# Lakonik/MVEdit

Measured on AMD Instinct MI355X. Metric: multi-view denoise-steps/sec (32 views, 512^2), higher is better.
Workload: dtype f16; 1 GPU; 32-view 512x512 get_noise_pred: 64 SD-1.5 UNet forwards (64x64 latents, ctx 77x768) + CFG per step; ControlNet residuals zero; views=32, latent=64, cfg=True, parallelism=views/1

## Files before the change

include/mvedit_amd.h:

```cpp
#ifndef MVEDIT_AMD_H
#define MVEDIT_AMD_H

#include <stdint.h>
#include <stddef.h>

#ifdef __cplusplus
extern "C" {
#endif

#define MVE_API __attribute__((visibility("default")))

typedef enum {
    MVE_OK = 0,
    MVE_ERR_ARG = -1,
    MVE_ERR_HIP = -2,
    MVE_ERR_STATE = -3,
    MVE_ERR_NOMEM = -4
} mve_status;

typedef enum {
    MVE_F32 = 0,
    MVE_F16 = 1,
    MVE_BF16 = 2,
    MVE_I32 = 3,
// ... 8 lines not shown
MVE_API int mve_near_far_from_aabb(const float* d_rays_o, const float* d_rays_d, const float* d_aabb,
                                   uint32_t N, float min_near, float* d_nears, float* d_fars, void* stream);

MVE_API int mve_morton3d(const int32_t* d_coords, uint32_t N, int32_t* d_indices, void* stream);
MVE_API int mve_morton3d_invert(const int32_t* d_indices, uint32_t N, int32_t* d_coords, void* stream);

MVE_API int mve_packbits(const float* d_grid, uint32_t n_bytes, float density_thresh, uint8_t* d_bitfield, void* stream);

MVE_API int mve_flatten_rays(const int32_t* d_rays, uint32_t N, uint32_t M, int32_t* d_res, void* stream);

MVE_API size_t mve_march_scratch_bytes(uint32_t N);
MVE_API int mve_march_rays_train_count(const float* d_rays_o, const float* d_rays_d, const uint8_t* d_grid,
                                       float bound, int contract, float dt_gamma, uint32_t max_steps,
                                       uint32_t N, uint32_t C, uint32_t H,
                                       const float* d_nears, const float* d_fars, const float* d_noises,
                                       int32_t* d_rays, int32_t* d_total, void* d_scratch, void* stream);
MVE_API int mve_march_rays_train_write(const float* d_rays_o, const float* d_rays_d, const uint8_t* d_grid,
                                       float bound, int contract, float dt_gamma, uint32_t max_steps,
                                       uint32_t N, uint32_t C, uint32_t H,
                                       const float* d_nears, const float* d_fars, const float* d_noises,
                                       const int32_t* d_rays, uint32_t capacity,
                                       float* d_xyzs, float* d_dirs, float* d_ts, void* stream);

MVE_API int mve_march_rays_train_clamp(const int32_t* d_rays, uint32_t N, const int32_t* d_total, uint32_t capacity,
                                       int32_t* d_n_samples, int32_t* d_count, int32_t* d_overflow, void* stream);

MVE_API int mve_composite_rays_train_forward(const float* d_sigmas, const float* d_rgbs, const float* d_ts,
                                             const int32_t* d_rays, uint32_t M, uint32_t N, float T_thresh, int binarize,
                                             float* d_weights, float* d_weights_sum, float* d_depth, float* d_image,
                                             void* stream);
MVE_API int mve_composite_rays_train_backward(const float* d_grad_weights, const float* d_grad_weights_sum,
                                              const float* d_grad_depth, const float* d_grad_image,
                                              const float* d_sigmas, const float* d_rgbs, const float* d_ts,
                                              const int32_t* d_rays, const float* d_weights_sum, const float* d_depth,
                                              const float* d_image, uint32_t M, uint32_t N, float T_thresh, int binarize,
                                              float* d_grad_sigmas, float* d_grad_rgbs, void* stream);

MVE_API int mve_march_rays(uint32_t n_alive, uint32_t n_step, const int32_t* d_rays_alive, const float* d_rays_t,
                           const float* d_rays_o, const float* d_rays_d, float bound, int contract, float dt_gamma,
                           uint32_t max_steps, uint32_t C, uint32_t H, const uint8_t* d_grid,
                           const float* d_nears, const float* d_fars,
                           float* d_xyzs, float* d_dirs, float* d_ts, const float* d_noises, void* stream);
MVE_API int mve_composite_rays(uint32_t n_alive, uint32_t n_step, float T_thresh, int binarize,
                               int32_t* d_rays_alive, float* d_rays_t, const float* d_sigmas, const float* d_rgbs,
                               const float* d_ts, float* d_weights_sum, float* d_depth, float* d_image, void* stream);

MVE_API int mve_compact_alive(const int32_t* d_rays_alive, uint32_t n_alive, int32_t* d_out, int32_t* d_n_out,
                              void* d_scratch, void* stream);

MVE_API size_t mve_cull_scratch_bytes(uint32_t M);
MVE_API int mve_cull_samples(const float* d_weights, uint32_t M, float threshold, const int32_t* d_rays, uint32_t N,
                             const float* d_xyzs, const float* d_dirs, const float* d_ts, float* d_out_xyzs, float* d_out_dirs,
                             float* d_out_ts, int32_t* d_out_rays, int32_t* d_pref, int32_t* d_n_out, void* d_scratch,
                             void* stream);
MVE_API int mve_cull_samples_n(const float* d_weights, uint32_t capacity, const int32_t* d_count, float threshold, const int32_t* d_rays,
                               uint32_t N, const float* d_xyzs, const float* d_dirs, const float* d_ts, float* d_out_xyzs,
                               float* d_out_dirs, float* d_out_ts, int32_t* d_out_rays, int32_t* d_pref, int32_t* d_n_out,
                               void* d_scratch, void* stream);

MVE_API int mve_density_grid_points(const int32_t* d_coords, const float* d_noise, uint32_t N, uint32_t grid_size, float bound,
                                    float* d_xyzs, int32_t* d_indices, void* stream);
MVE_API size_t mve_density_grid_scratch_bytes(uint32_t n_cells);
MVE_API int mve_density_grid_update(float* d_density_grid, float* d_tmp_grid, uint32_t n_cells, const float* d_sigmas,
                                    const int32_t* d_indices, uint32_t N, float decay, float* d_mean_density, void* d_scratch,
                                    void* stream);


#define MVE_GEMM_GEGLU   1
#define MVE_GEMM_OUT_F32 2
#define MVE_CONV_W_CHUNK64 4
#define MVE_GEMM_NO_SPLITK 8
#define MVE_CONV_PAD_BR 32
#define MVE_GEMM_RES_AFTER_SCALE 16

MVE_API int mve_gemm(int dtype, const void* d_A, int lda, const void* d_W, int ldw, void* d_out, int ldc,
                     int M, int N, int K, const float* d_bias, const float* d_rowvec, int ldrv, int rows_per_vec,
                     const void* d_residual, int ldr, int flags, float out_scale, void* d_workspace,
                     size_t workspace_bytes, int rows_per_image, void* stream);

MVE_API int mve_gemm_tune(int big_min_blocks);
MVE_API int mve_gemm_red_tune(int on);
MVE_API int mve_gemm_deep_tune(int max_blocks);
MVE_API int mve_gemm_effective_splitk(int M, int N, int K, int rows_per_image);
#define MVE_PLAN_RESIDUAL 1
#define MVE_PLAN_RESIDUAL_LO 2
#define MVE_PLAN_OUT_LO 4
#define MVE_PLAN_ROWVEC 8
#define MVE_PLAN_LN 16
#define MVE_PLAN_BIAS 32
#define MVE_PLAN_WORKSPACE 64
#define MVE_PLAN_SCALED 128
#define MVE_PLAN_DESCRIBE_INTS 12
MVE_API int mve_gemm_plan_describe(int kind, int M, int N, int K, int rows_per_image, int flags, int features, const int* conv_geom, int* out);

MVE_API int mve_gemm_pp_profile(void* d_buf);

MVE_API size_t mve_gemm_workspace_bytes(int M, int N, int K, int rows_per_image);

MVE_API int mve_conv3x3(int dtype, const void* d_x1, int C1, const void* d_x2, int C2, int B, int Hs, int Ws,
                        int stride, int upsample, const void* d_W, int Cout, void* d_out, int ldc,
                        const float* d_bias, const float* d_rowvec, int ldrv, const void* d_residual, int ldr,
                        int flags, float out_scale, void* d_workspace, size_t workspace_bytes, void* stream);

MVE_API int mve_conv3x3_shortcut(int dtype, const void* x1, int C1, const void* x3, int C3, const void* x4, int C4, int B, int Hs,
                                 int Ws, const void* W, int Cout, void* out, int ldc, const float* bias, const float* bias2,
                                 const void* residual, int ldr, int flags, float out_scale, void* d_workspace,
                                 size_t workspace_bytes, void* stream);

MVE_API int mve_upsample_conv_phases_supported(int C, int Cout, int B, int Hs, int Ws);
MVE_API int mve_upsample_conv_phases_tune(int one_launch);
MVE_API size_t mve_upsample_conv_phases_workspace_bytes(int C, int Cout, int B, int Hs, int Ws);
MVE_API int mve_pack_upsample_phase_weights(int src_dtype, int dst_dtype, const void* d_w_oihw, int Cout, int C, void* d_W4, void* stream);
MVE_API int mve_upsample_conv_phases(int dtype, const void* d_x, int C, int B, int Hs, int Ws, const void* d_W4, int Cout, void* d_out,
                                     const float* d_bias, int flags, void* d_workspace, size_t workspace_bytes, void* d_out_lo, void* stream);

MVE_API int mve_gemm_pair(int dtype, const void* d_A, int lda, const void* d_W, int ldw, void* d_out, int ldc,
                          int M, int N, int K, const float* d_bias, const float* d_rowvec, int ldrv, int rows_per_vec,
                          const void* d_residual, int ldr, int flags, float out_scale, void* d_workspace,
                          size_t workspace_bytes, int rows_per_image, const void* d_residual_lo, void* d_out_lo, void* stream);

MVE_API int mve_gemm_pair_ln(int dtype, const void* d_A, int lda, const void* d_W, int ldw, void* d_out, int ldc, int M, int N, int K,
                             const float* d_bias, const void* d_residual, int ldr, void* d_workspace, size_t workspace_bytes, int rows_per_image,
                             const void* d_residual_lo, void* d_out_lo, void* d_ln_out, int ld_ln, const float* d_ln_gamma, const float* d_ln_beta,
                             float ln_eps, void* stream);
MVE_API int mve_gemm_ln_fuse_tune(int on);

MVE_API int mve_conv3x3_pair(int dtype, const void* x1, int C1, const void* x2, int C2, int B, int Hs, int Ws, int stride,
                             int upsample, const void* W, int Cout, void* out, int ldc, const float* bias, const float* rowvec,
                             int ldrv, const void* residual, int ldr, int flags, float out_scale, void* d_workspace,
                             size_t workspace_bytes, const void* d_residual_lo, void* d_out_lo, void* stream);
MVE_API int mve_conv3x3_shortcut_pair(int dtype, const void* x1, int C1, const void* x3, int C3, const void* x4, int C4, int B, int Hs,
                                      int Ws, const void* W, int Cout, void* out, int ldc, const float* bias, const float* bias2,
                                      int flags, float out_scale, void* d_workspace, size_t workspace_bytes, void* d_out_lo, void* stream);
MVE_API int mve_groupnorm_silu_pair(int dtype, const void* d_x1, int C1, const void* d_x2, int C2, int B, int HW, int G,
                                    float eps, const float* d_gamma, const float* d_beta, int silu, void* d_out,
                                    void* d_workspace, const void* d_x1_lo, const void* d_x2_lo, void* stream);
MVE_API int mve_layernorm_pair(int dtype, const void* d_x, int ldx, void* d_y, int ldy, int M, int C,
                               const float* d_gamma, const float* d_beta, float eps, const void* d_x_lo, void* stream);
MVE_API int mve_axpy_pair(int dtype, const void* d_a, const void* d_a_lo, const void* d_b, float alpha, void* d_y, void* d_y_lo, size_t n, void* stream);

MVE_API int mve_mxfp8_packed_k(int K);
MVE_API int mve_mxfp8_quantize(int dtype, const void* d_x, int ldx, int R, int K, uint8_t* d_q, uint8_t* d_e, void* stream);
MVE_API int mve_mxfp8_gemm(const uint8_t* d_aq, const uint8_t* d_ae, const uint8_t* d_wq, const uint8_t* d_we, int M, int N, int K, int out_dtype,
                           void* d_out, int ldc, const float* d_bias, const void* d_residual, int ldr, void* stream);

MVE_API int mve_attention(int dtype, const void* d_Q, int ldq, const void* d_K, int ldk, const void* d_V, int ldv,
                          const void* d_K2, int ldk2, const void* d_V2, int ldv2, void* d_O, int ldo,
                          int B, int Lq, int Lk, int Lk2, int heads, int head_dim, float scale, void* stream);
MVE_API int mve_attention_tune(int variant);
MVE_API int mve_attention_profile(unsigned long long* out4);
MVE_API int mve_attention_prescaled(int dtype, const void* d_Q, int ldq, const void* d_K, int ldk, const void* d_V, int ldv,
                                    const void* d_K2, int ldk2, const void* d_V2, int ldv2, void* d_O, int ldo,
                                    int B, int Lq, int Lk, int Lk2, int heads, int head_dim, void* stream);


MVE_API int mve_attention_causal(int dtype, const void* d_Q, int ldq, const void* d_K, int ldk, const void* d_V, int ldv, void* d_O, int ldo,
                                 int B, int L, int heads, int head_dim, float scale, void* stream);
MVE_API int mve_clip_embed(int dtype, const int32_t* d_ids, const void* d_tok, const void* d_pos, void* d_out, int B, int L, int C, int vocab,
                           int max_pos, void* stream);
#define MVE_ACT_QUICK_GELU 0
#define MVE_ACT_GELU 1
MVE_API int mve_act(int dtype, int kind, const void* d_x, void* d_y, size_t n, void* stream);
MVE_API int mve_clip_pool(int dtype, const void* d_x, const int32_t* d_ids, void* d_out, int B, int L, int C, int eos_token_id, void* stream);


MVE_API int mve_clip_patchify(int dtype, const void* d_pixels, int B, int H, int W, int P, void* d_rows, int ld, void* stream);
MVE_API int mve_clip_vision_embed(int dtype, const void* d_patch, const void* d_cls, const void* d_pos, void* d_out, int B, int G2, int C, void* stream);


MVE_API int mve_dpt_stem_rows(int dtype, const void* d_pixels, int B, int S, void* d_rows, int ld, void* stream);
MVE_API int mve_dpt_maxpool(int dtype, const void* d_x, int B, int H, int W, int C, void* d_y, void* stream);
MVE_API int mve_dpt_gather_s2(int dtype, const void* d_x, int B, int H, int W, int C, void* d_y, void* stream);
MVE_API int mve_dpt_upsample2x(int dtype, const void* d_x, int B, int H, int W, int C, void* d_y, void* stream);
MVE_API int mve_dpt_add_relu(int dtype, const void* d_a, const void* d_b, void* d_y, size_t n, void* stream);


MVE_API int mve_loftr_stem_rows(int dtype, const void* d_pixels, int B, int H, int W, void* d_rows, int ld, void* stream);
MVE_API int mve_loftr_leaky_relu(int dtype, const void* d_x, void* d_y, size_t n, float slope, void* stream);
MVE_API int mve_loftr_pos_add(int dtype, const void* d_x, const float* d_pos, void* d_y, int B, int HW, int C, void* stream);

MVE_API size_t mve_linattn_workspace_bytes(int B, int S, int H, int D);
MVE_API int mve_linattn_kv(int dtype, const void* d_k, int ldk, const void* d_v, int ldv, int B, int S, int H, int D, float* d_kv, void* d_workspace,
                           size_t workspace_bytes, void* stream);
MVE_API int mve_linattn_apply(int dtype, const void* d_q, int ldq, const float* d_kv, void* d_out, int ldo, int B, int L, int H, int D, float eps,
                              void* stream);

MVE_API int mve_dsmax_stats(const float* d_sim, int N, int L, int S, int ld, float* d_row_stats, float* d_col_stats, void* stream);
MVE_API int mve_dsmax_conf(const float* d_sim, int N, int L, int S, int ld, const float* d_row_stats, const float* d_col_stats, float* d_conf, void* stream);
MVE_API size_t mve_dsmax_select_workspace_bytes(int N, int L, int S);
MVE_API int mve_dsmax_select(const float* d_conf, int N, int H0, int W0, int H1, int W1, float thr, int border, float scale, int64_t* d_b_ids,
                             int64_t* d_i_ids, int64_t* d_j_ids, float* d_mconf, float* d_mkpts0_c, float* d_mkpts1_c, int* d_count, void* d_workspace,
                             size_t workspace_bytes, void* stream);

MVE_API int mve_loftr_unfold(int dtype, const void* d_feat, int N, int Hf, int Wf, int C, const int64_t* d_b_ids, const int64_t* d_ids, int M, void* d_rows,
                             void* stream);
MVE_API int mve_loftr_ln_add(int dtype, const void* d_o, int ldo, const void* d_x, int ldx, void* d_y, int ldy, int M, int C, const float* d_gamma,
                             const float* d_beta, float eps, void* stream);
MVE_API int mve_loftr_gather_rows(int dtype, const void* d_feat, int N, int L, int C, const int64_t* d_b_ids, const int64_t* d_ids, int M, void* d_rows,
                                  void* stream);
MVE_API int mve_loftr_fine_match(int dtype, const void* d_feat0, const void* d_feat1, int M, int C, const float* d_mkpts1_c, float radius, float* d_expec_f,
                                 float* d_mkpts1_f, void* stream);


MVE_API int mve_attention_relpos(int dtype, const void* d_Q, int ldq, const void* d_K, int ldk, const void* d_V, int ldv, const void* d_rel_h,
                                 const void* d_rel_w, void* d_O, int ldo, int NS, int gh, int gw, int heads, int head_dim, float scale, void* stream);
MVE_API int mve_sam_window_partition(int dtype, const void* d_x, int B, int G, int C, int window, void* d_win, void* stream);
MVE_API int mve_sam_window_unpartition(int dtype, const void* d_win, int B, int G, int C, int window, void* d_x, void* stream);
MVE_API int mve_sam_pos_add(int dtype, const void* d_x, const void* d_pos, void* d_y, int B, int HW, int C, void* stream);

MVE_API int mve_groupnorm_tune(int fused_max_hw);
MVE_API size_t mve_groupnorm_workspace_bytes(int B, int HW, int C, int G);
MVE_API int mve_groupnorm_silu(int dtype, const void* d_x1, int C1, const void* d_x2, int C2, int B, int HW, int G,
                               float eps, const float* d_gamma, const float* d_beta, int silu, void* d_out,
                               void* d_workspace, void* stream);

MVE_API int mve_layernorm(int dtype, const void* d_x, int ldx, void* d_y, int ldy, int M, int C,
                          const float* d_gamma, const float* d_beta, float eps, void* stream);

MVE_API int mve_nchw_to_nhwc(int dst_dtype, int src_dtype, const void* d_x, int B, int C, int H, int W, int Cpad,
                             void* d_y, void* stream);
MVE_API int mve_nhwc_to_nchw(int dst_dtype, int src_dtype, const void* d_x, int ld, int B, int C, int H, int W,
                             void* d_y, void* stream);
MVE_API int mve_timestep_embedding(int dtype, const float* d_t, int B, int dim, void* d_out, void* stream);
MVE_API int mve_text_time_embedding(int dtype, const void* d_text_embeds, int text_dtype, int text_dim, const float* d_time_ids, int n_ids,
                                    int time_embed_dim, int B, void* d_out, void* stream);
MVE_API int mve_silu(int dtype, const void* d_x, void* d_y, size_t n, void* stream);
MVE_API int mve_axpy(int dtype, const void* d_a, const void* d_b, float alpha, void* d_y, size_t n, void* stream);
MVE_API int mve_softmax_rows(int dtype, const float* d_scores, size_t lds, int M, int N, void* d_probs, size_t ldp, void* stream);
MVE_API int mve_cfg_combine(const float* d_uncond, const float* d_text, float guidance_scale, float* d_out, size_t n,
                            void* stream);
MVE_API int mve_x0_prediction(const float* d_latents_scaled, const float* d_noise_pred, float sqrt_alpha_bar,
                              float sqrt_one_minus_alpha_bar, size_t n, float* d_x0, void* stream);

MVE_API int mve_tonemap_lut(const float* d_x, size_t n, const float* d_lut_x, const float* d_lut_y, int steps, int inverse, int linear,
                            float* d_out, void* stream);
MVE_API int mve_tonemap_lut_backward(const float* d_x, const float* d_grad_out, size_t n, const float* d_lut_x, const float* d_lut_y,
                                     int steps, int inverse, int linear, float* d_grad_x, void* stream);

MVE_API int mve_gaussian_blur(const float* d_x, int planes, int H, int W, int ksize, float sigma, int adjoint, const float* d_base,
                              float offset, float* d_tmp, float* d_out, void* stream);

MVE_API int mve_sh_encode(const float* d_inputs, uint32_t B, int degree, float* d_outputs, float* d_dy_dx, void* stream);
MVE_API int mve_sh_encode_backward(const float* d_grad, const float* d_dy_dx, uint32_t B, int degree, float* d_grad_inputs, void* stream);
MVE_API int mve_shade_views(const float* d_rgba, const float* d_normal_fg, const float* d_cam_lights, uint32_t n_views,
                            uint32_t pix_per_view, float ambient_light, float bg_color, const float* d_lut_x, const float* d_lut_y,
                            int steps, float* d_image, void* stream);
MVE_API int mve_shade_points(const float* d_albedo, const float* d_normal, const float* d_lights, size_t N, float ambient_light,
                             const float* d_lut_x, const float* d_lut_y, int steps, float* d_out, const float* d_grad_out,
                             float* d_grad_albedo, float* d_grad_normal, void* stream);

typedef struct MveReconLossDesc {
    int32_t P, ps, shaded, is_init, lut_steps;
    float ambient_light, bg_color, normal_bg[3];
    float pixel_loss_weight, normal_reg_weight, depth_weight, entropy_weight, bg_width;
    const float *d_lut_x, *d_lut_y;
    const float *d_image, *d_weights_sum, *d_depth;
    const float *d_weights, *d_ts;
    uint32_t M;
    const float *d_target_dir, *d_target_rgbs, *d_target_m, *d_target_n, *d_target_depth;
    const float *d_patch_w, *d_patch_lights;
} MveReconLossDesc;
MVE_API size_t mve_recon_loss_workspace_bytes(int P, int ps, uint32_t M);
MVE_API int mve_recon_loss_forward(const MveReconLossDesc* desc, void* d_ws, size_t ws_bytes, float* d_losses, float* d_out_rgbs,
                                   float* d_out_normals, void* stream);
MVE_API int mve_recon_loss_backward(const MveReconLossDesc* desc, void* d_ws, size_t ws_bytes, const float* d_g_out_rgbs,
                                    const float* d_g_out_normals, const float* d_g_loss, float* d_g_image, float* d_g_weights_sum, float* d_g_depth,
                                    float* d_g_weights, void* stream);
MVE_API int mve_recon_loss_forward_n(const MveReconLossDesc* desc, const int32_t* d_count, void* d_ws, size_t ws_bytes, float* d_losses,
                                     float* d_out_rgbs, float* d_out_normals, void* stream);
MVE_API int mve_recon_loss_backward_n(const MveReconLossDesc* desc, const int32_t* d_count, void* d_ws, size_t ws_bytes,
                                      const float* d_g_out_rgbs, const float* d_g_out_normals, const float* d_g_loss, float* d_g_image,
                                      float* d_g_weights_sum, float* d_g_depth, float* d_g_weights, void* stream);

typedef struct MveMeshLossDesc {
    int32_t n, size, mesh_is_simplified;
    float normal_bg[3];
    float pixel_loss_weight, normal_reg_weight;
    const float *d_rgba, *d_normal, *d_depth;
    const float *d_target_dir, *d_target_rgbs, *d_target_m_erode, *d_target_m_blur, *d_target_n;
    const float *d_view_w;
} MveMeshLossDesc;
MVE_API size_t mve_mesh_loss_workspace_bytes(int n, int size);
MVE_API int mve_mesh_loss_forward(const MveMeshLossDesc* desc, void* d_ws, size_t ws_bytes, float* d_losses, float* d_out_rgbs,
                                  float* d_out_normals, void* stream);
MVE_API int mve_mesh_loss_backward(const MveMeshLossDesc* desc, void* d_ws, size_t ws_bytes, const float* d_g_out_rgbs,
                                   const float* d_g_out_normals, const float* d_g_loss, float* d_g_rgba, float* d_g_normal, void* stream);

MVE_API size_t mve_mesh_reg_workspace_bytes(int V, int F);
MVE_API int mve_mesh_reg_forward(const float* d_verts, int V, const int32_t* d_faces, int F, const float* d_face_normals, void* d_ws,
                                 size_t ws_bytes, float* d_losses, void* stream);
MVE_API int mve_mesh_reg_backward(const float* d_verts, int V, const int32_t* d_faces, int F, const float* d_face_normals, void* d_ws,
                                  size_t ws_bytes, const float* d_g_losses, float* d_g_verts, float* d_g_face_normals, void* stream);

MVE_API int mve_mesh_normals_forward(const float* d_verts, int V, const int32_t* d_faces, int F, float* d_face_normals, float* d_vn_sum,
                                     float* d_vn, void* stream);
MVE_API int mve_mesh_normals_backward(const float* d_verts, int V, const int32_t* d_faces, int F, const float* d_vn_sum, const float* d_g_vn,
                                      const float* d_g_face_normals, float* d_scratch, float* d_g_verts, void* stream);

MVE_API int mve_unet_create(void** handle, int dtype, int in_channels, int out_channels, int n_levels,
                            const int* block_out_channels, int layers_per_block, const int* down_attn,
                            const int* num_heads, const int* transformer_layers, int cross_attention_dim,
                            int norm_num_groups, float norm_eps, int use_linear_projection);
MVE_API int mve_unet_destroy(void* handle);
MVE_API size_t mve_unet_weight_bytes(void* handle);
MVE_API int mve_unet_load_param(void* handle, const char* name, const void* d_src, int src_dtype, int ndim,
                                const long long* shape, void* stream);
// ... 312 lines not shown
```

mvedit_amd/build.py:

```python
import concurrent.futures as cf
import hashlib
import json
import os
import shutil
import subprocess
import sys

ROOT = os.path.dirname(os.path.abspath(__file__))
REPO = os.path.dirname(ROOT)
CSRC = os.path.join(ROOT, 'csrc')
OBJDIR = os.path.join(ROOT, '_build')
LIB = os.path.join(ROOT, 'libmvedit_amd.so')
ARCH = 'gfx950'

COMMON_FLAGS = [
    f'--offload-arch={ARCH}', '-O3', '-std=c++17', '-fPIC', '-fvisibility=hidden',
    '-Wall', '-Wno-unused-function', '-Wno-unknown-pragmas',
    '-I' + os.path.join(REPO, 'include'),
]
EXTRA_FLAGS = {
    'attention.hip': ['-fno-honor-nans'],
    'raymarching.hip': ['-ffp-contract=off'],
    'nerf.hip': ['-ffp-contract=off'],
    'hashgrid_encode.hip': ['-ffp-contract=off'],
    'raster.hip': ['-ffp-contract=off'],
    'dmtet.hip': ['-ffp-contract=off'],
    'shading.hip': ['-ffp-contract=off'],
    'recon_loss.hip': ['-ffp-contract=off'],
    'mesh_reg.hip': ['-ffp-contract=off'],
    'blur.hip': ['-ffp-contract=off'],
    'sh.hip': ['-ffp-contract=off'],
    'triplane.hip': ['-ffp-contract=off'],
    'texture_grad.hip': ['-ffp-contract=off'],
}


_TAG = os.environ.get('MVE_BUILD_TAG', '')
if _TAG:
    OBJDIR = os.path.join(ROOT, '_build_' + _TAG)
    LIB = os.path.join(ROOT, f'libmvedit_amd_{_TAG}.so')
    COMMON_FLAGS = COMMON_FLAGS + ['-D' + d for d in os.environ.get('MVE_BUILD_DEFS', '').split(',') if d]

if os.environ.get('MVE_ATTN_LAB') == '1':
    EXTRA_FLAGS['attention.hip'] = EXTRA_FLAGS['attention.hip'] + ['-DMVE_ATTN_LAB']


def _hipcc():
    for cand in (os.environ.get('HIPCC'), shutil.which('hipcc'), '/opt/rocm/bin/hipcc'):
        if cand and os.path.exists(cand):
            return cand
    raise RuntimeError('hipcc not found (set HIPCC)')


def _sources():
    return sorted(f for f in os.listdir(CSRC) if f.endswith(('.hip', '.cpp')))


def _headers_digest():
    h = hashlib.sha256()
    for d in (CSRC, os.path.join(REPO, 'include')):
        for f in sorted(os.listdir(d)):
            if f.endswith(('.h', '.hpp', '.inc')):
                with open(os.path.join(d, f), 'rb') as fh:
                    h.update(f.encode())
                    h.update(fh.read())
    return h.hexdigest()


_INC_RE = None


def _deps_digest(path, seen=None):
    global _INC_RE
    import re
    if _INC_RE is None:
        _INC_RE = re.compile(r'^\s*#\s*include\s*"([^"]+)"', re.M)
    seen = seen if seen is not None else {}
    if path in seen:
        return ''
    seen[path] = True
    with open(path, 'rb') as fh:
        data = fh.read()
    h = hashlib.sha256(data)
    for inc in _INC_RE.findall(data.decode('utf-8', 'replace')):
        for d in (os.path.dirname(path), CSRC, os.path.join(REPO, 'include')):
            cand = os.path.join(d, inc)
            if os.path.exists(cand):
                h.update(_deps_digest(cand, seen).encode())
                break
    return h.hexdigest()


def _compile_one(hipcc, src, hdr_digest, verbose):
    path = os.path.join(CSRC, src)
    hdr_digest = _deps_digest(path)
    obj = os.path.join(OBJDIR, src + '.o')
    stamp = obj + '.stamp'
    flags = COMMON_FLAGS + EXTRA_FLAGS.get(src, [])
    with open(path, 'rb') as fh:
        key = hashlib.sha256(fh.read() + hdr_digest.encode() + json.dumps(flags).encode()).hexdigest()
    if os.path.exists(obj) and os.path.exists(stamp) and open(stamp).read() == key:
        return obj, False
    cmd = [hipcc] + flags + (['-x', 'hip'] if src.endswith('.cpp') else []) + ['-c', path, '-o', obj]
    if verbose:
        print(' '.join(cmd), flush=True)
    r = subprocess.run(cmd, capture_output=True, text=True)
    if r.returncode != 0:
        raise RuntimeError(f'hipcc failed on {src}:\n{r.stdout}\n{r.stderr}')
    if r.stderr.strip() and verbose:
        print(r.stderr, file=sys.stderr)
    with open(stamp, 'w') as fh:
        fh.write(key)
    return obj, True


def build(verbose=False, force=False):
    hipcc = _hipcc()
    os.makedirs(OBJDIR, exist_ok=True)
    if force:
        for f in os.listdir(OBJDIR):
            os.remove(os.path.join(OBJDIR, f))
    hdr = _headers_digest()
    srcs = _sources()
    objs, rebuilt = [], False
    with cf.ThreadPoolExecutor(max_workers=min(8, os.cpu_count() or 1)) as ex:
        for obj, changed in ex.map(lambda s: _compile_one(hipcc, s, hdr, verbose), srcs):
            objs.append(obj)
            rebuilt |= changed
    if rebuilt or not os.path.exists(LIB):
        cmd = [hipcc, f'--offload-arch={ARCH}', '-shared', '-fPIC', '-o', LIB] + objs
        if verbose:
            print(' '.join(cmd), flush=True)
        r = subprocess.run(cmd, capture_output=True, text=True)
        if r.returncode != 0:
            raise RuntimeError(f'link failed:\n{r.stdout}\n{r.stderr}')
    return LIB


if __name__ == '__main__':
    print(build(verbose=True, force='--force' in sys.argv))
```

mvedit_amd/csrc/attention.hip:

```cpp
#include "common.h"

#include <stdlib.h>
#include <type_traits>

namespace {

constexpr int NT = 256;

struct AttnParams {
    const void* Q; const void* K; const void* V; const void* K2; const void* V2; void* O;
    int ldq, ldk, ldv, ldk2, ldv2, ldo;
    int B, Lq, Lk, Lk2, heads;
    float scale_log2e;
    int prescaled;
    const int* skip_if;
};

template <int DP, bool KSW2> __device__ __forceinline__ int k_perm(int row, int pc) {
    if constexpr (DP == 64) return pc ^ ((row >> 1) & 7);
    else if constexpr (KSW2) return pc ^ (((row >> 3) & 1) << 1);
    else return pc ^ ((row >> 2) & 3);
}
template <int DP, bool KSW2> __device__ __forceinline__ int k_swz(int row, int chunk) {
    return row * (DP * 2) + (k_perm<DP, KSW2>(row, chunk) << 4);
// ... 556 lines not shown
                if constexpr (PRE && (ABL & 8) != 0) {
                    e0 = sk[2 * r2]; e1 = sk[2 * r2 + 1];
                } else if constexpr (PRE) {
                    e0 = __builtin_amdgcn_exp2f(sk[2 * r2]);
                    e1 = __builtin_amdgcn_exp2f(sk[2 * r2 + 1]);
                } else {
                    e0 = __builtin_amdgcn_exp2f(__builtin_fmaf(sk[2 * r2], sc, nm));
                    e1 = __builtin_amdgcn_exp2f(__builtin_fmaf(sk[2 * r2 + 1], sc, nm));
                }
                pk[r2] = __builtin_bit_cast(unsigned, __builtin_convertvector(f32x2{e0, e1}, T2));
            }
#pragma unroll
            for (int v = 0; v < 4; ++v) {
                const int ai = v < 2 ? v : v + 2;
                if constexpr ((ABL & 512) != 0) { pb.w[kb][0][v] = pk[ai]; pb.w[kb][1][v] = pk[ai + 2]; continue; }
                const auto r = __builtin_amdgcn_permlane16_swap(pk[ai], pk[ai + 2], false, false);
                pb.w[kb][0][v] = r[0];
                pb.w[kb][1][v] = r[1];
            }
        }
        return pb;
    };

    auto pv = [&](const unsigned char* St, const PB& pb) {
#pragma unroll
        for (int kb = 0; kb < 2; ++kb) {
            s16x4 lo[3], up[3];
            const unsigned va0 = (unsigned)(uintptr_t)(lds_ptr_t)(St + v_off + kb * 32 * V_ROW);
            if constexpr ((ABL & 256) != 0) {
#pragma unroll
                for (int i = 0; i < 3; ++i) { lo[i] = __builtin_bit_cast(s16x4, u32x2{pb.w[kb][0][i], va0}); up[i] = __builtin_bit_cast(s16x4, u32x2{va0, pb.w[kb][1][i]}); }
            } else {
                typedef __attribute__((address_space(3))) s16x4* lp;
#pragma unroll
                for (int i = 0; i < 3; ++i) {
                    lo[i] = __builtin_amdgcn_ds_read_tr16_b64_v4i16((lp)(lds_ptr_t)(St + v_off + kb * 32 * V_ROW + 32 * i));
                    up[i] = __builtin_amdgcn_ds_read_tr16_b64_v4i16((lp)(lds_ptr_t)(St + v_off + kb * 32 * V_ROW + 32 * i + 16 * V_ROW));
                }
            }
#pragma unroll
            for (int i = 0; i < 3; ++i) {
                const V8 va = __builtin_bit_cast(V8, __builtin_shufflevector(lo[i], up[i], 0, 1, 2, 3, 4, 5, 6, 7));
#pragma unroll
                for (int f = 0; f < 2; ++f) {
                    const u32x4 pw = {pb.w[kb][f][0], pb.w[kb][f][1], pb.w[kb][f][2], pb.w[kb][f][3]};
                    if constexpr ((ABL & 64) != 0) { asm volatile("" : "+v"(oacc[i][f]) : "v"(va), "v"(pw)); continue; }
                    oacc[i][f] = Tag::mfma16(va, __builtin_bit_cast(V8, pw), oacc[i][f]);
                }
            }
        }
    };

    auto wait_sync = [&](int keep) {
        if constexpr ((ABL & 3) == 3) { asm volatile("s_waitcnt lgkmcnt(0)" ::: "memory"); return; }
        else if constexpr ((ABL & 1) != 0) { asm volatile("s_waitcnt vmcnt(0)\n\ts_waitcnt lgkmcnt(0)" ::: "memory"); return; }
        else if constexpr ((ABL & 2) != 0) { asm volatile("s_waitcnt lgkmcnt(0)\n\ts_barrier" ::: "memory"); return; }
        if (keep >= 3) asm volatile("s_waitcnt vmcnt(3)\n\ts_waitcnt lgkmcnt(0)\n\ts_barrier" ::: "memory");
        else if (keep == 2) asm volatile("s_waitcnt vmcnt(2)\n\ts_waitcnt lgkmcnt(0)\n\ts_barrier" ::: "memory");
        else if (keep == 1) asm volatile("s_waitcnt vmcnt(1)\n\ts_waitcnt lgkmcnt(0)\n\ts_barrier" ::: "memory");
        else asm volatile("s_waitcnt vmcnt(0)\n\ts_waitcnt lgkmcnt(0)\n\ts_barrier" ::: "memory");
    };
    auto next_stage = [&](int off) { return off + STAGE == NST * STAGE ? 0 : off + STAGE; };

    if constexpr (!PIPE) {
        constexpr int PD = NST - 1;
        static_assert(DMA_PER_WAVE * (PD - 1) <= 3, "wait_sync covers at most three outstanding instructions");
#pragma unroll
        for (int i = 0; i < PD; ++i)
            if (i < n_tiles) dma(i, i * STAGE);
        asm volatile("" : "+v"(qf[0]), "+v"(qf[1]), "+v"(qf[2]));
        wait_sync(n_mine * ((n_tiles < PD ? n_tiles : PD) - 1));
        int cur = 0, nxt = PD * STAGE;
        for (int t = 0; t < n_full; ++t) {
            if (t + PD < n_tiles) dma(t + PD, nxt);
            S2 s = qk(smem + cur);
            softmax_max(s, t * KB, std::false_type{}, t == 0);
            const PB pb = softmax_exp(s);
            pv(smem + cur, pb);
            const int last_issued = t + PD < n_tiles ? t + PD : n_tiles - 1;
            wait_sync(last_issued > t + 1 ? n_mine * (last_issued - (t + 1)) : 0);
            nxt = cur;
            cur = next_stage(cur);
        }
        if (n_full < n_tiles) {
            S2 s = qk(smem + cur);
            softmax_max(s, n_full * KB, std::true_type{}, n_full == 0);
            const PB pb = softmax_exp(s);
            pv(smem + cur, pb);
        }
    } else {
        static_assert(NST >= 3, "the pipelined loop needs the next tile's K resident");
        constexpr int PD = NST - 1;
        static_assert(DMA_PER_WAVE * (PD - 2) <= 3, "wait_sync covers at most three outstanding instructions");
#pragma unroll
        for (int i = 0; i < PD; ++i)
            if (i < n_tiles) dma(i, i * STAGE);
        asm volatile("" : "+v"(qf[0]), "+v"(qf[1]), "+v"(qf[2]));
        {
            const int issued = n_tiles < PD ? n_tiles : PD;
            wait_sync(issued > 2 ? n_mine * (issued - 2) : 0);
        }
        int cur = 0, nx1 = STAGE, nxt = (PD % NST) * STAGE;
        S2 sA = qk(smem), sB;
        const int n_main = n_tiles - 1;
        auto step = [&](S2& sc_, S2& sn_, int t) {
            if (t + PD < n_tiles) dma(t + PD, nxt);
            softmax_max(sc_, t * KB, std::false_type{}, t == 0);
            sn_ = qk(smem + nx1);
            const PB pb = softmax_exp(sc_);
            pv(smem + cur, pb);
            const int last_issued = t + PD < n_tiles ? t + PD : n_tiles - 1;
            wait_sync(last_issued > t + 2 ? n_mine * (last_issued - (t + 2)) : 0);
            nxt = cur; cur = nx1; nx1 = next_stage(nx1);
        };
        int t = 0;
        for (; t + 2 <= n_main; t += 2) { step(sA, sB, t); step(sB, sA, t + 1); }
        if (t < n_main) { step(sA, sB, t); sA = sB; ++t; }
        if (n_full < n_tiles) softmax_max(sA, t * KB, std::true_type{}, t == 0);
        else softmax_max(sA, t * KB, std::false_type{}, t == 0);
        const PB pb = softmax_exp(sA);
        pv(smem + cur, pb);
    }

#pragma unroll
    for (int f = 0; f < 2; ++f) {
        const float l = __shfl(oacc[2][f][0], 32 + l16, 64);
        const float inv = 1.0f / l;
        const int q = q_base + f * 16 + l16;
        if (q < p.Lq) {
            T* orow = reinterpret_cast<T*>(p.O) + ((size_t)b * p.Lq + q) * p.ldo + h * D;
#pragma unroll
            for (int i = 0; i < 3; ++i) {
                const int dv = i * 16 + g * 4;
                if (dv < D) {
                    T4 o4;
#pragma unroll
                    for (int r = 0; r < 4; ++r) o4[r] = Tag::from_f32(oacc[i][f][r] * inv);
                    *reinterpret_cast<T4*>(orow + dv) = o4;
                }
            }
        }
    }
    if constexpr ((ABL & 1024) != 0) {
        unsigned long long t1, r1;
        asm volatile("s_memtime %0\n\ts_memrealtime %1\n\ts_waitcnt lgkmcnt(0)" : "=s"(t1), "=s"(r1) :: "memory");
        if (lane == 0 && (blockIdx.x & 63) == 5) {
            atomicAdd(&g_attn_prof[0], t1 - prof_t0);
            atomicAdd(&g_attn_prof[1], r1 - prof_r0);
            atomicAdd(&g_attn_prof[2], 1ull);
        }
    }
}

int g_attn_variant = 9;
int g_attn_ablate = 0;

template <class Tag, int D>
int launch(const AttnParams& p, hipStream_t s) {
    if constexpr (D == 40) {
        if (g_attn_variant >= 8 && g_attn_variant <= 15) {
            const int var = g_attn_variant;
            const bool w8 = var == 9 || var == 11 || var >= 14;
            const unsigned grid3 = (unsigned)(((p.Lq + (w8 ? 255 : 127)) / (w8 ? 256 : 128)) * p.heads * p.B);
#define MVE_A3P(SEG, NW_, NST_, WPS_, PRE_, PIPE_) k_attention3<Tag, SEG, NW_, NST_, WPS_, PRE_, PIPE_><<<grid3, 64 * NW_, 0, s>>>(p)
#define MVE_A3(NW_, NST_, WPS_, PIPE_) do { \
                if (p.Lk2 > 0) { if (p.prescaled && !PIPE_) MVE_A3P(true, NW_, NST_, WPS_, (!PIPE_), PIPE_); else MVE_A3P(true, NW_, NST_, WPS_, false, PIPE_); } \
                else { if (p.prescaled && !PIPE_) MVE_A3P(false, NW_, NST_, WPS_, (!PIPE_), PIPE_); else MVE_A3P(false, NW_, NST_, WPS_, false, PIPE_); } } while (0)
#ifdef MVE_ATTN_LAB
            if (g_attn_ablate != 0) {
                if constexpr (std::is_same<Tag, F16Tag>::value) {
                    if (p.Lk2 == 0 && p.prescaled) {
                        const unsigned grid9 = (unsigned)(((p.Lq + 255) / 256) * p.heads * p.B);
                        bool hit = true;
                        switch (g_attn_ablate) {
#define MVE_ABL(A) case A: k_attention3<Tag, false, 8, 2, 4, true, false, (A) | 1024><<<grid9, 512, 0, s>>>(p); break;
                            MVE_ABL(2048) MVE_ABL(1) MVE_ABL(3) MVE_ABL(7) MVE_ABL(8) MVE_ABL(16) MVE_ABL(24) MVE_ABL(32) MVE_ABL(64) MVE_ABL(96) MVE_ABL(128) MVE_ABL(256)
                            MVE_ABL(384) MVE_ABL(512) MVE_ABL(536) MVE_ABL(927) MVE_ABL(480) MVE_ABL(1023)
#undef MVE_ABL
                            default: hit = false;
                        }
                        if (hit) { MVE_LAUNCH_CHECK(); return MVE_OK; }
                    }
                }
            }
#endif
            switch (var) {
                case 8: MVE_A3(4, 2, 4, false); break;
                case 9: MVE_A3(8, 2, 4, false); break;
                case 10: MVE_A3(4, 3, 4, false); break;
                case 11: MVE_A3(8, 3, 4, false); break;
                case 12: MVE_A3(4, 3, 3, true); break;
                case 13: MVE_A3(4, 4, 3, true); break;
                case 14: MVE_A3(8, 3, 2, true); break;
                default: MVE_A3(8, 4, 2, true); break;
            }
#undef MVE_A3P
#undef MVE_A3
            MVE_LAUNCH_CHECK();
            return MVE_OK;
        }
        if (g_attn_variant == 1 && p.Lk2 == 0) {
            const unsigned grid1 = (unsigned)(((p.Lq + 63) / 64) * p.heads * p.B);
            k_attention2<Tag, D, false, 1, 64, 3><<<grid1, NT, 0, s>>>(p);
            MVE_LAUNCH_CHECK();
            return MVE_OK;
        }
    }
    constexpr int QB = 128;
    const unsigned grid = (unsigned)(((p.Lq + QB - 1) / QB) * p.heads * p.B);
    const int var = g_attn_variant >= 8 ? ((D == 80 || D == 160) ? 6 : 4) : g_attn_variant;
    if constexpr (D == 80 || D == 160) {
        if ((var == 2 || var == 6) && p.Lk2 == 0) {
            if (var == 6) k_attention2<Tag, D, false, 2, 0, 0, true, true><<<grid, NT, 0, s>>>(p);
            else k_attention2<Tag, D, false, 2, 0, 0, true><<<grid, NT, 0, s>>>(p);
            MVE_LAUNCH_CHECK();
            return MVE_OK;
        }
    }
    if ((var == 4 || var == 6) && p.Lk2 == 0) {
        k_attention2<Tag, D, false, 2, 0, 0, false, true><<<grid, NT, 0, s>>>(p);
        MVE_LAUNCH_CHECK();
        return MVE_OK;
    }
    if (p.Lk2 > 0) k_attention2<Tag, D, true><<<grid, NT, 0, s>>>(p);
    else k_attention2<Tag, D, false><<<grid, NT, 0, s>>>(p);
    MVE_LAUNCH_CHECK();
    return MVE_OK;
}

template <class Tag>
int dispatch_d(const AttnParams& p, int d, hipStream_t s) {
    switch (d) {
        case 40: return launch<Tag, 40>(p, s);
        case 64: return launch<Tag, 64>(p, s);
        case 80: return launch<Tag, 80>(p, s);
        case 160: return launch<Tag, 160>(p, s);
        default:
            mve_set_error("attention: unsupported head dim %d (supported: 40, 64, 80, 160)", d);
            return MVE_ERR_ARG;
    }
}

}

extern "C" int mve_attention_profile(unsigned long long* out4) {
    MVE_CHECK(out4, MVE_ERR_ARG, "attention_profile: null pointer");
#ifndef MVE_ATTN_LAB
    mve_set_error("attention_profile: the timing-only ablation kernels are compiled into development builds only (MVE_ATTN_LAB=1 python -m mvedit_amd.build)");
    return MVE_ERR_STATE;
#endif
    MVE_HIP(hipDeviceSynchronize());
    MVE_HIP(hipMemcpyFromSymbol(out4, HIP_SYMBOL(g_attn_prof), 4 * sizeof(unsigned long long)));
    const unsigned long long z[4] = {0ull, 0ull, 0ull, 0ull};
    MVE_HIP(hipMemcpyToSymbol(HIP_SYMBOL(g_attn_prof), z, sizeof(z)));
    return MVE_OK;
}

extern "C" int mve_attention_tune(int variant) {
    const int old = g_attn_variant | (g_attn_ablate << 8);
#ifndef MVE_ATTN_LAB
    if (variant >= 256) { mve_set_error("attention_tune: ablation bits (8-19) need a development build (MVE_ATTN_LAB=1)"); return MVE_ERR_ARG; }
#endif
    if (variant >= 0) { g_attn_variant = variant & 255; g_attn_ablate = (variant >> 8) & 4095; }
    return old;
}

static int attention_entry(int dtype, const void* Q, int ldq, const void* K, int ldk, const void* V, int ldv,
                           const void* K2, int ldk2, const void* V2, int ldv2, void* O, int ldo, int B, int Lq,
                           int Lk, int Lk2, int heads, int head_dim, float scale, int prescaled, void* stream) {
    if (B == 0 || Lq == 0) return MVE_OK;
    MVE_CHECK(Q && K && V && O, MVE_ERR_ARG, "attention: null pointer");
    MVE_CHECK(Lk > 0 && Lk2 >= 0 && heads > 0, MVE_ERR_ARG, "attention: bad sizes Lk=%d Lk2=%d heads=%d", Lk, Lk2, heads);
    MVE_CHECK(Lk2 == 0 || (K2 && V2), MVE_ERR_ARG, "attention: second KV segment has null pointers");
    MVE_CHECK(ldq % 8 == 0 && ldk % 8 == 0 && ldv % 8 == 0 && ldo % 4 == 0 && (Lk2 == 0 || (ldk2 % 8 == 0 && ldv2 % 8 == 0)),
              MVE_ERR_ARG, "attention: leading dimensions must be multiples of 8");
    AttnParams p;
    p.Q = Q; p.K = K; p.V = V; p.K2 = K2; p.V2 = V2; p.O = O;
    p.ldq = ldq; p.ldk = ldk; p.ldv = ldv; p.ldk2 = ldk2; p.ldv2 = ldv2; p.ldo = ldo;
    p.B = B; p.Lq = Lq; p.Lk = Lk; p.Lk2 = Lk2; p.heads = heads;
    p.scale_log2e = prescaled ? 1.0f : scale * 1.4426950408889634f;
    p.prescaled = prescaled;
    p.skip_if = mve_skip_second_half();
    MVE_CHECK(!p.skip_if || B % 2 == 0, MVE_ERR_ARG, "attention: the second-half predicate needs an even batch (B=%d)", B);
    if (dtype == MVE_F16) return dispatch_d<F16Tag>(p, head_dim, (hipStream_t)stream);
    if (dtype == MVE_BF16) return dispatch_d<BF16Tag>(p, head_dim, (hipStream_t)stream);
    mve_set_error("attention: unsupported dtype %d", dtype);
    return MVE_ERR_ARG;
}

extern "C" int mve_attention(int dtype, const void* Q, int ldq, const void* K, int ldk, const void* V, int ldv,
                             const void* K2, int ldk2, const void* V2, int ldv2, void* O, int ldo, int B, int Lq,
                             int Lk, int Lk2, int heads, int head_dim, float scale, void* stream) {
    return attention_entry(dtype, Q, ldq, K, ldk, V, ldv, K2, ldk2, V2, ldv2, O, ldo, B, Lq, Lk, Lk2, heads, head_dim, scale, 0, stream);
}

extern "C" int mve_attention_prescaled(int dtype, const void* Q, int ldq, const void* K, int ldk, const void* V, int ldv,
                                       const void* K2, int ldk2, const void* V2, int ldv2, void* O, int ldo, int B, int Lq,
                                       int Lk, int Lk2, int heads, int head_dim, void* stream) {
    return attention_entry(dtype, Q, ldq, K, ldk, V, ldv, K2, ldk2, V2, ldv2, O, ldo, B, Lq, Lk, Lk2, heads, head_dim, 1.0f, 1, stream);
}
```

Before: 16.54 denoise-steps/s.

## Add register-resident short-KV attention kernel for cross-attention (Lk<=96)

Adds a dedicated attention kernel for short key sequences such as the 77-token text context. All K and V fragments for a head stay in registers, several heads are packed per block, and Q tiles are staged through shared memory with a one-tile global prefetch. Softmax is done in a single pass without online rescaling, and the output is written back through the same tile. The kernel is on by default and can be disabled with an env var. Separately, the build skips recompiling when a tree digest stamp matches.

```diff
diff --git a/include/mvedit_amd.h b/include/mvedit_amd.h
--- a/include/mvedit_amd.h
+++ b/include/mvedit_amd.h
@@ -184,6 +184,7 @@
 MVE_API int mve_attention_prescaled(int dtype, const void* d_Q, int ldq, const void* d_K, int ldk, const void* d_V, int ldv,
                                     const void* d_K2, int ldk2, const void* d_V2, int ldv2, void* d_O, int ldo,
                                     int B, int Lq, int Lk, int Lk2, int heads, int head_dim, void* stream);
+MVE_API int mve_attention_short_tune(int on);
 
 
 MVE_API int mve_attention_causal(int dtype, const void* d_Q, int ldq, const void* d_K, int ldk, const void* d_V, int ldv, void* d_O, int ldo,
diff --git a/mvedit_amd/build.py b/mvedit_amd/build.py
--- a/mvedit_amd/build.py
+++ b/mvedit_amd/build.py
@@ -114,6 +114,14 @@
     return obj, True
 
 
+def _tree_digest(srcs):
+    h = hashlib.sha256()
+    for s in srcs:
+        flags = [f.replace(REPO, '.') for f in COMMON_FLAGS + EXTRA_FLAGS.get(s, [])]
+        h.update((s + _deps_digest(os.path.join(CSRC, s)) + json.dumps(flags)).encode())
+    return h.hexdigest()
+
+
 def build(verbose=False, force=False):
     hipcc = _hipcc()
     os.makedirs(OBJDIR, exist_ok=True)
@@ -122,6 +130,9 @@
             os.remove(os.path.join(OBJDIR, f))
     hdr = _headers_digest()
     srcs = _sources()
+    lib_stamp, digest = os.path.join(OBJDIR, 'lib.stamp'), _tree_digest(srcs)
+    if os.path.exists(LIB) and os.path.exists(lib_stamp) and open(lib_stamp).read() == digest:
+        return LIB
     objs, rebuilt = [], False
     with cf.ThreadPoolExecutor(max_workers=min(8, os.cpu_count() or 1)) as ex:
         for obj, changed in ex.map(lambda s: _compile_one(hipcc, s, hdr, verbose), srcs):
@@ -134,6 +145,8 @@
         r = subprocess.run(cmd, capture_output=True, text=True)
         if r.returncode != 0:
             raise RuntimeError(f'link failed:\n{r.stdout}\n{r.stderr}')
+    with open(lib_stamp, 'w') as fh:
+        fh.write(digest)
     return LIB
 
 
diff --git a/mvedit_amd/csrc/attention.hip b/mvedit_amd/csrc/attention.hip
--- a/mvedit_amd/csrc/attention.hip
+++ b/mvedit_amd/csrc/attention.hip
@@ -732,11 +732,251 @@
     }
 }
 
+constexpr int SHORT_LK = 96;
+
+constexpr int short_blocks_per_cu(int d, int kf) { return d == 40 && kf <= 5 ? 3 : 2; }
+
+template <class Tag, int D, int G, int R, int KF>
+__global__ __launch_bounds__(64 * G, short_blocks_per_cu(D, KF)) void k_attention_short(const AttnParams p, const int tiles_per_block) {
+    constexpr int NTH = 64 * G;
+    constexpr int KK = (KF + 1) / 2;
+    constexpr int KFM = KF == 6 ? 5 : KF == 5 ? 2 : 0;
+    constexpr bool QPF = D == 64;
+    constexpr int DP = (D + 31) / 32 * 32, KS = DP / 32, DC = D / 8, DVF = (D + 15) / 16;
+    constexpr int CPR = G * D / 8;
+    constexpr int ROWB = CPR * 16 + 16;
+    constexpr int NV = (R * CPR + NTH - 1) / NTH;
+    constexpr int RF = R / 16;
+    typedef typename Tag::V8 V8;
+    typedef typename Tag::T T;
+    typedef T T4 __attribute__((ext_vector_type(4)));
+
+    __shared__ __attribute__((aligned(16))) unsigned char tile[R * ROWB];
+
+    const int tid = threadIdx.x, lane = tid & 63, wid = __builtin_amdgcn_readfirstlane(tid >> 6);
+    const int g = lane >> 4, l16 = lane & 15;
+
+    const int n_tiles = (p.Lq + R - 1) / R;
+    const int chunks = (n_tiles + tiles_per_block - 1) / tiles_per_block;
+    const int groups = (p.heads + G - 1) / G;
+    const unsigned nblk = (unsigned)(chunks * groups * p.B);
+    const unsigned bid = p.skip_if ? mve_xcd_remap_halves(blockIdx.x, nblk, nblk / 2) : mve_xcd_remap(blockIdx.x, nblk);
+    const int grp = bid % groups;
+    const int ch = (bid / groups) % chunks;
+    const int b = bid / (groups * chunks);
+    if (mve_second_half_skipped(p.skip_if, 2 * b >= p.B)) return;
+
+    const int h0 = grp * G;
+    const int nh = p.heads - h0 < G ? p.heads - h0 : G;
+    const int cpr = nh * DC;
+    const bool active = wid < nh;
+    const int Lk = p.Lk;
+
+    V8 kfr[KF][KS], vfr[DVF][KK];
+    {
+        const int h = active ? h0 + wid : h0;
+        const T* kb = reinterpret_cast<const T*>(p.K) + (size_t)b * Lk * p.ldk + h * D;
+        const unsigned short* vb = reinterpret_cast<const unsigned short*>(p.V) + (size_t)b * Lk * p.ldv + h * D;
+#pragma unroll
+        for (int kf = 0; kf < KF; ++kf) {
+            const int key = kf * 16 + l16;
+            const int keyc = key < Lk ? key : Lk - 1;
+#pragma unroll
+            for (int ks = 0; ks < KS; ++ks) {
+                const int c = ks * 4 + g;
+                const u32x4 v = *reinterpret_cast<const u32x4*>(kb + (size_t)keyc * p.ldk + (c < DC ? c : DC - 1) * 8);
+                kfr[kf][ks] = __builtin_bit_cast(V8, (key < Lk && c < DC) ? v : u32x4{0u, 0u, 0u, 0u});
+            }
+        }
+#pragma unroll
+        for (int i = 0; i < DVF; ++i) {
+            const int dv = i * 16 + l16;
+            const int dvc = dv < D ? dv : D - 1;
+#pragma unroll
+            for (int kk = 0; kk < KK; ++kk) {
+                u16x8 v;
+#pragma unroll
+                for (int e = 0; e < 8; ++e) {
+                    const int key = (2 * kk + (e >> 2)) * 16 + 4 * g + (e & 3);
+                    const u16 x = vb[(size_t)(key < Lk ? key : Lk - 1) * p.ldv + dvc];
+                    v[e] = (dv < D && key < Lk) ? x : (u16)0;
+                }
+                vfr[i][kk] = __builtin_bit_cast(V8, v);
+            }
+#pragma unroll
+            for (int kk = 0; kk < KK; ++kk) asm volatile("" : "+v"(vfr[i][kk]));
+        }
+    }
+    V8 ones;
+#pragma unroll
+    for (int e = 0; e < 8; ++e) ones[e] = Tag::from_f32(1.0f);
+
+    const unsigned char* Qg = reinterpret_cast<const unsigned char*>(p.Q) + ((size_t)b * p.Lq * p.ldq + h0 * D) * 2;
+    unsigned char* Og = reinterpret_cast<unsigned char*>(p.O) + ((size_t)b * p.Lq * p.ldo + h0 * D) * 2;
+    int c_row[NV], c_col[NV];
+#pragma unroll
+    for (int i = 0; i < NV; ++i) {
+        const int idx = tid + i * NTH;
+        const int row = idx / CPR, c = idx - row * CPR;
+        const bool ok = idx < R * CPR && c < cpr;
+        c_row[i] = ok ? row : -1;
+        c_col[i] = ok ? c * 16 : 0;
+    }
+    u32x4 pre[NV];
+    auto gload = [&](int t) {
+#pragma unroll
+        for (int i = 0; i < NV; ++i) {
+            int q = t * R + (c_row[i] >= 0 ? c_row[i] : 0);
+            q = q < p.Lq ? q : p.Lq - 1;
+            pre[i] = *reinterpret_cast<const u32x4*>(Qg + (size_t)q * p.ldq * 2 + c_col[i]);
+        }
+    };
+    auto landed = [&]() {
+#pragma unroll
+        for (int i = 0; i < NV; ++i) asm volatile("" : "+v"(pre[i]));
+    };
+    auto load_q = [&](int f, V8 (&qf)[KS]) {
+        const unsigned char* qrow = tile + (f * 16 + l16) * ROWB + wid * (D * 2);
+#pragma unroll
+        for (int ks = 0; ks < KS; ++ks) {
+            const int c = ks * 4 + g;
+            const u32x4 v = *reinterpret_cast<const u32x4*>(qrow + (c < DC ? c : DC - 1) * 16);
+            qf[ks] = __builtin_bit_cast(V8, c < DC ? v : u32x4{0u, 0u, 0u, 0u});
+        }
+    };
+
+    const float sc = p.scale_log2e;
+    const int lim = Lk - 4 * g;
+    const int t_end = (ch + 1) * tiles_per_block < n_tiles ? (ch + 1) * tiles_per_block : n_tiles;
+    int t = ch * tiles_per_block;
+    if (t < t_end) { gload(t); landed(); }
+    for (; t < t_end; ++t) {
+#pragma unroll
+        for (int i = 0; i < NV; ++i)
+            if (c_row[i] >= 0) *reinterpret_cast<u32x4*>(tile + c_row[i] * ROWB + c_col[i]) = pre[i];
+        __syncthreads();
+        if (t + 1 < t_end) gload(t + 1);
+
+        if (active) {
+            V8 qn[KS];
+            if constexpr (QPF) load_q(0, qn);
+#pragma unroll 1
+            for (int f = 0; f < RF; ++f) {
+                unsigned char* qrow = tile + (f * 16 + l16) * ROWB + wid * (D * 2);
+                V8 qf[KS];
+                if constexpr (QPF) {
+#pragma unroll
+                    for (int ks = 0; ks < KS; ++ks) qf[ks] = qn[ks];
+                    load_q((f + 1) & (RF - 1), qn);
+                } else {
+                    load_q(f, qf);
+                }
+                f32x4 s[KF];
+                float mx = -INFINITY;
+#pragma unroll
+                for (int kf = 0; kf < KF; ++kf) {
+                    s[kf] = f32x4{0.f, 0.f, 0.f, 0.f};
+#pragma unroll
+                    for (int ks = 0; ks < KS; ++ks) s[kf] = Tag::mfma16(kfr[kf][ks], qf[ks], s[kf]);
+                    if (kf >= KFM) {
+#pragma unroll
+                        for (int r = 0; r < 4; ++r) s[kf][r] = kf * 16 + r < lim ? s[kf][r] : -INFINITY;
+                    }
+#pragma unroll
+                    for (int r = 0; r < 4; ++r) mx = fmaxf(mx, s[kf][r]);
+                }
+                mx = mve_max_xor32(mve_max_xor16(mx));
+                const float mxs = mx * sc;
+                V8 pf[KK];
+#pragma unroll
+                for (int kk = 0; kk < KK; ++kk) {
+                    f32x8 e;
+#pragma unroll
+                    for (int r = 0; r < 4; ++r) {
+                        e[r] = __builtin_amdgcn_exp2f(__builtin_fmaf(s[2 * kk][r], sc, -mxs));
+                        e[4 + r] = 2 * kk + 1 < KF ? __builtin_amdgcn_exp2f(__builtin_fmaf(s[2 * kk + 1 < KF ? 2 * kk + 1 : 0][r], sc, -mxs)) : 0.f;
+                    }
+                    pf[kk] = __builtin_convertvector(e, V8);
+                }
+                f32x4 oacc[DVF], lacc = f32x4{0.f, 0.f, 0.f, 0.f};
+#pragma unroll
+                for (int i = 0; i < DVF; ++i) oacc[i] = f32x4{0.f, 0.f, 0.f, 0.f};
+#pragma unroll
+                for (int kk = 0; kk < KK; ++kk) {
+#pragma unroll
+                    for (int i = 0; i < DVF; ++i) oacc[i] = Tag::mfma16(vfr[i][kk], pf[kk], oacc[i]);
+                    lacc = Tag::mfma16(ones, pf[kk], lacc);
+                }
+                const float inv = 1.0f / lacc[0];
+#pragma unroll
+                for (int i = 0; i < DVF; ++i) {
+                    const int dv = i * 16 + g * 4;
+                    if (dv < D) {
+                        T4 o4;
+#pragma unroll
+                        for (int r = 0; r < 4; ++r) o4[r] = Tag::from_f32(oacc[i][r] * inv);
+                        *reinterpret_cast<T4*>(qrow + dv * 2) = o4;
+                    }
+                }
+            }
+        }
+        __syncthreads();
+        landed();
+#pragma unroll
+        for (int i = 0; i < NV; ++i) {
+            const int q = t * R + c_row[i];
+            if (c_row[i] >= 0 && q < p.Lq)
+                *reinterpret_cast<u32x4*>(Og + (size_t)q * p.ldo * 2 + c_col[i]) = *reinterpret_cast<const u32x4*>(tile + c_row[i] * ROWB + c_col[i]);
+        }
+        __syncthreads();
+    }
+}
+
+int g_attn_short = -1;
+bool attn_short_enabled() {
+    if (g_attn_short < 0) {
+        const char* e = getenv("MVE_ATTN_SHORT");
+        g_attn_short = (e && e[0] == '0' && e[1] == 0) ? 0 : 1;
+    }
+    return g_attn_short != 0;
+}
+
+template <int D>
+bool attn_short_takes(const AttnParams& p) {
+    if constexpr (D == 40 || D == 64 || D == 80)
+        return p.Lk2 == 0 && p.Lk <= SHORT_LK && p.ldo % 8 == 0 && (reinterpret_cast<uintptr_t>(p.O) & 15) == 0 &&
+               (reinterpret_cast<uintptr_t>(p.Q) & 15) == 0;
+    return false;
+}
+
+template <class Tag, int D>
+int launch_short(const AttnParams& p, hipStream_t s) {
+    constexpr int G = D == 64 ? 5 : 4;
+    constexpr int R = D == 40 ? 64 : 32;
+    const int n_tiles = (p.Lq + R - 1) / R, groups = (p.heads + G - 1) / G;
+    const int kf = p.Lk <= 32 ? 2 : p.Lk <= 80 ? 5 : 6;
+    const long long pairs = (long long)p.B * groups;
+    long long want = (256 * short_blocks_per_cu(D, kf) + pairs - 1) / pairs;
+    if (want < 1) want = 1;
+    if (want > n_tiles) want = n_tiles;
+    const int tpb = (n_tiles + (int)want - 1) / (int)want;
+    const int chunks = (n_tiles + tpb - 1) / tpb;
+    const unsigned grid = (unsigned)(chunks * groups * p.B);
+    if (kf == 2) k_attention_short<Tag, D, G, R, 2><<<grid, 64 * G, 0, s>>>(p, tpb);
+    else if (kf == 5) k_attention_short<Tag, D, G, R, 5><<<grid, 64 * G, 0, s>>>(p, tpb);
+    else k_attention_short<Tag, D, G, R, 6><<<grid, 64 * G, 0, s>>>(p, tpb);
+    MVE_LAUNCH_CHECK();
+    return MVE_OK;
+}
+
 int g_attn_variant = 9;
 int g_attn_ablate = 0;
 
 template <class Tag, int D>
 int launch(const AttnParams& p, hipStream_t s) {
+    if constexpr (D == 40 || D == 64 || D == 80) {
+        if (attn_short_enabled() && attn_short_takes<D>(p)) return launch_short<Tag, D>(p, s);
+    }
     if constexpr (D == 40) {
         if (g_attn_variant >= 8 && g_attn_variant <= 15) {
             const int var = g_attn_variant;
@@ -845,6 +1085,12 @@
     return old;
 }
 
+extern "C" int mve_attention_short_tune(int on) {
+    const int old = attn_short_enabled() ? 1 : 0;
+    if (on >= 0) g_attn_short = on ? 1 : 0;
+    return old;
+}
+
 static int attention_entry(int dtype, const void* Q, int ldq, const void* K, int ldk, const void* V, int ldv,
                            const void* K2, int ldk2, const void* V2, int ldv2, void* O, int ldo, int B, int Lq,
                            int Lk, int Lk2, int heads, int head_dim, float scale, int prescaled, void* stream) {
```

Result: no change. 16.66 denoise-steps/s (median of 6 runs) (+0.8%).
